# tprelle/janusgraph

Measured on AMD Instinct MI355X. Metric: GTEPS for PageRank iter + BFS, RMAT-24/26, 1/2/4/8 GPUs; % of HBM peak, higher is better.
Workload: dtype f64

## Files before the change

janusgraph_amd/csrc/jg_api.cpp:

```cpp
#include <dlfcn.h>
#include <execinfo.h>

#include <algorithm>
#include <atomic>
#include <cstdlib>
#include <cstring>
#include <limits>
#include <map>
#include <mutex>

#include "jg_cache.h"
#include "jg_internal.h"
#include "jg_labelset.h"

namespace jg {

namespace {
thread_local std::string g_last_error;
}

void rccl_check(ncclResult_t r, const char* what) {
    if (r != ncclSuccess) fail(JG_ERR_RCCL, std::string(what) + ": " + ncclGetErrorString(r));
}

// ... 595 lines not shown
    bool sealed = false;
    jg::DevBuf<int64_t> lab;
    int64_t ml = 0;
};

using jg::Error;

#define JG_GUARD_BEGIN try {
#define JG_GUARD_END                                       \
    jg::dev_cache_sync();                                  \
    return JG_OK;                                          \
    }                                                      \
    catch (const Error& e) {                               \
        jg::g_last_error_set(e.what());                    \
        return e.code;                                     \
    }                                                      \
    catch (const std::bad_alloc&) {                        \
        jg::g_last_error_set("host allocation failed");    \
        return JG_ERR_OOM;                                 \
    }                                                      \
    catch (const std::exception& e) {                      \
        jg::g_last_error_set(e.what());                    \
        return JG_ERR_HIP;                                 \
    }

namespace jg {
void g_last_error_set(const char* m) { g_last_error = m ? m : ""; }
}

#define JG_ARG(cond, msg) \
    if (!(cond)) jg::fail(JG_ERR_ARG, msg)

extern "C" {

int jg_abi_version(void) { return JG_ABI_VERSION; }

int jg_tune_set(const char* key, int64_t value) {
    JG_GUARD_BEGIN
    JG_ARG(key, "null key");
    const std::string k(key);
    jg::Tune& t = jg::tune();
    if (k == "dev_poison_probe") {
        jg::dev_poison_probe(value);
        return JG_OK;
    }
    struct Knob {
        const char* name;
        int* field;
        int64_t lo, hi;
    };
    const Knob knobs[] = {
        {"pull_split", &t.pull_split, 0, 1},
        {"halo", &t.halo, 0, 1},
        {"bfs_alpha", &t.bfs_alpha, 1, 1000000},
        {"dobfs_alpha", &t.dobfs_alpha, 1, 1000000},
        {"bfs_beta", &t.bfs_beta, 1, 1000000},
        {"bfs_narrow", &t.bfs_narrow, 0, 1},
        {"nb_alpha", &t.nb_alpha, 1, 1000000},
        {"nb_first", &t.nb_first, 4, 4096},
        {"cc_push", &t.cc_push, 0, 1},
        {"msbfs_sparse", &t.msbfs_sparse, 0, 1},
        {"msbfs_td", &t.msbfs_td, 0, 2},
        {"cc_first", &t.cc_first, 1, 64},
        {"msbfs_skip", &t.msbfs_skip, 0, 1},
        {"msbfs_exit", &t.msbfs_exit, 0, 2},
        {"msbfs_td_rowapply", &t.msbfs_td_rowapply, 0, 1024},
        {"msbfs_td_noprobe", &t.msbfs_td_noprobe, 0, 1000},
        {"msbfs_scan_queue", &t.msbfs_scan_queue, 0, 1001},
        {"msbfs_exit_first", &t.msbfs_exit_first, 1, 256},
        {"msbfs_exit_live", &t.msbfs_exit_live, 0, 1000},
        {"cc_uf", &t.cc_uf, 0, 1},
        {"cc_uf_sharded", &t.cc_uf_sharded, 0, 1},
        {"cc_uf_search", &t.cc_uf_search, 0, 1},
        {"cc_sparse", &t.cc_sparse, 0, 1},
        {"msbfs_split", &t.msbfs_split, 0, 1},
        {"sharded_bfs", &t.sharded_bfs, 0, 1},
        {"bfs_td_split", &t.bfs_td_split, 0, 2},
        {"bfs_td_split_levels", &t.bfs_td_split_levels, 0, 0xffff},
        {"bfs_batch0", &t.bfs_batch0, 1, 64},
        {"bfs_grid_mult", &t.bfs_grid_mult, 1, 64},
        {"bfs_grid", &t.bfs_grid, 64, 65536},
        {"bfs_tail_grid", &t.bfs_tail_grid, 0, 65536},
        {"merge_temporal", &t.merge_temporal, 0, 2},
        {"sd_delta", &t.sd_delta, -1, 1 << 30},
        {"sd_dist32", &t.sd_dist32, 0, 2},
    };
    for (const Knob& kn : knobs) {
        if (k != kn.name) continue;
        if (value < kn.lo || value > kn.hi)
            jg::fail(JG_ERR_ARG, k + " must be in [" + std::to_string(kn.lo) + ", " + std::to_string(kn.hi) + "]");
        *kn.field = (int)value;
        return JG_OK;
    }
    if (k.rfind("band", 0) == 0 && k.size() == 9 && k[4] >= '0' && k[4] <= '3' &&
        (k.substr(5) == "_deg" || k.substr(5) == "_bit" || k.substr(5) == "_sub")) {
        const int i = k[4] - '0';
        if (k.substr(5) == "_deg") {
            JG_ARG(value >= -1, "band degree must be >= 0 (0: unused) or -1 (automatic)");
            t.band_deg[i] = value;
        } else if (k.substr(5) == "_bit") {
            JG_ARG(value == 0 || (value >= 3 && value <= 8), "band bits must be 0 (automatic) or in [3, 8]");
            t.band_bits[i] = value == 0 ? -1 : (int)value;
        } else {
            JG_ARG(value >= 1 && value <= 256 && (value & (value - 1)) == 0, "band sub-slices must be a power of two in [1, 256]");
            int b = 0;
            while ((1 << b) < value) ++b;
            t.band_bits[i] = b;
        }
    } else if (k.size() == 12 && k.compare(0, 11, "merge_stage") == 0 && k[11] >= '0' && k[11] <= '3') {
        JG_ARG(value == -1 || value == 0 || value == 64 || value == 128 || value == 256 || value == 512,
               "merge_stage<i> must be -1 (automatic), 0, 64, 128, 256 or 512");
        t.merge_stage[k[11] - '0'] = (int)value;
    } else if (k == "bfs_td_split_min" || k == "bfs_td_split_max") {
        JG_ARG(value >= 1 && value <= INT32_MAX, "bfs_td_split_min / _max must be in [1, 2^31)");
        (k == "bfs_td_split_min" ? t.bfs_td_split_min : t.bfs_td_split_max) = value;
    } else if (k == "merge_pack") {
        JG_ARG(value == 0 || value == 1 || value == 24, "merge_pack must be 0 (32 bits), 1 (automatic) or 24 (at least 24)");
        t.merge_pack = (int)value;
    } else if (k == "pull_unroll" || k == "pull_nt" || k == "pull_lds" || k == "light_lds" || k == "slice_lds" ||
               k == "pull_short" || k == "pull_overlap" || k == "bfs_persistent") {
    } else {
        jg::fail(JG_ERR_ARG, "unknown tuning key: " + k);
    }
    JG_GUARD_END
}

const char* jg_last_error(void) { return jg::g_last_error.c_str(); }

int jg_comm_unique_id(void* out) {
    JG_GUARD_BEGIN
    JG_ARG(out, "null output");
    ncclUniqueId id;
    jg::rccl_check(ncclGetUniqueId(&id), "ncclGetUniqueId");
    static_assert(sizeof(ncclUniqueId) == JG_UNIQUE_ID_BYTES, "unique id size");
    std::memcpy(out, &id, sizeof id);
    JG_GUARD_END
}

int jg_ctx_create(const int* devices, int ndev, jg_ctx** out) {
    JG_GUARD_BEGIN
    JG_ARG(out && devices && ndev > 0, "jg_ctx_create: need devices and an output pointer");
    *out = nullptr;
    int count = 0;
    JG_HIP(hipGetDeviceCount(&count));
    for (int i = 0; i < ndev; ++i)
        JG_ARG(devices[i] >= 0 && devices[i] < count, "jg_ctx_create: device ordinal out of range");
    auto ctx = std::make_unique<jg_ctx>();
    jg::Ctx& c = ctx->impl;
    c.devices.assign(devices, devices + ndev);
    bool all_same = true;
    for (int i = 1; i < ndev; ++i) all_same &= devices[i] == devices[0];
    c.logical = ndev > 1 && all_same;
    jg::vdev_refresh();
    jg::dev_poison_refresh();
    c.vdev = c.logical && jg::vdev_mode() != 0;
    if (ndev > 1 && !all_same) {
        std::vector<int> sorted(c.devices);
        std::sort(sorted.begin(), sorted.end());
        JG_ARG(std::adjacent_find(sorted.begin(), sorted.end()) == sorted.end(),
               "jg_ctx_create: mix of repeated and distinct devices");
    }
    for (int i = 0; i < ndev; ++i) {
        jg::DeviceGuard dg(c.devices[i]);
        hipStream_t s = nullptr;
        if (c.logical && i > 0) s = c.streams[0];
        else JG_HIP(hipStreamCreateWithFlags(&s, hipStreamNonBlocking));
// ... 804 lines not shown
```

janusgraph_amd/csrc/jg_internal.h:

```cpp
#pragma once

#include <algorithm>
#include <memory>
#include <atomic>
#include <mutex>
#include <functional>
#include <vector>

#include "jg_common.h"
#include "janusgpu.h"

#include <rccl/rccl.h>

namespace jg {

struct Csr {
    int64_t rows = 0;
    int64_t nnz = 0;
    DevBuf<int64_t> row_ptr;
    DevBuf<int32_t> col;
    DevBuf<int32_t> weight;
    mutable int64_t empty_from = -1;
    mutable DevBuf<int32_t> first_col;
    mutable long long wstat[4] = {0, 0, 0, 0};
// ... 404 lines not shown
void graph_neighbors(const Graph& g, int direction, const int64_t* rows, int64_t nrows, int64_t* off_out,
                     int64_t* nbr_out);
void shortest_distance_run(Graph& g, int64_t seed_vid, int max_depth, int64_t* dist_out);
using CcLabelHook = std::function<void(const int32_t* label, int64_t lrows)>;
void cc_run(Graph& g, int64_t* comp_out, int32_t* iterations_out, const CcLabelHook* labels_hook = nullptr);
void cc_census(Graph& g, int64_t min_population, int32_t* iterations_out, int64_t* components_out, int64_t* listed_out,
               int64_t* largest_out, double* census_ms_out);
void cc_census_read(Graph& g, int64_t first, int64_t count, int64_t* vid_out, int64_t* pop_out);
void cc_census_drop(Graph& g);
void cc_prepare_ranks(Graph& g);
struct CcRoots {
    int32_t* parent;
    const int32_t* rank;
    const int32_t* minr;
    int64_t ne;
};
int cc_root_eccentricity(Ctx& ctx, Shard& sh, const CcRoots& r, int32_t* depth, double* edges_out,
                         const std::function<void()>* after_start = nullptr, hipEvent_t end_ev = nullptr);
int cc_root_eccentricity_sharded(Graph& g, const CcRoots* roots, double* edges_out);
void bfs_buffers(Shard& sh);
const int32_t* bfs_first_col(Shard& sh, const Csr& c);
void region_mark(hipStream_t s, bool begin);
constexpr int kNarrowMax = 8;
struct NarrowRun {
    int levels = 0;
    float ms = 0;
    double entries = 0;
    double bytes = 0;
    double reached = 0;
};
NarrowRun narrow_bfs(Ctx& ctx, Shard& sh, const Csr& push, const Csr& pull, const int64_t* src, int ns, int max_depth,
                     int32_t* planes);
void combine_run(Graph& g, int direction, int combiner, int wrap32, const int64_t* init, int steps, int64_t* out,
                 uint8_t* received_out);

int allreduce_or(Graph& g, int flag);
void allreduce_sum_i64(Graph& g, int64_t* vals, int n);
uint64_t allreduce_or_u64(Graph& g, uint64_t v);

bool pull_split_launches();
bool debug_plan();
bool debug_bfs();

struct Tune {
    int pull_split = 1;
    int64_t band_deg[4] = {96, -1, -1, 0};
    int band_bits[4] = {-1, -1, -1, 3};
    int halo = 1;
    int bfs_alpha = 14;
    int dobfs_alpha = 30;
    int bfs_beta = 24;
    int bfs_narrow = 1;
    int nb_alpha = 30;
    int nb_first = 16;
    int cc_push = 1;
    int msbfs_sparse = 1;
    int msbfs_td = 1;
    int cc_first = 1;
    int msbfs_skip = 1;
    int msbfs_exit = 1;
    int msbfs_td_rowapply = 4;
    int msbfs_td_noprobe = 2;
    int msbfs_scan_queue = 50;
    int msbfs_exit_first = 16;
    int msbfs_exit_live = 950;
    int cc_uf = 1;
    int cc_uf_sharded = 1;
    int cc_uf_search = 1;
    int cc_sparse = 1;
    int msbfs_split = 1;
    int sharded_bfs = 1;
    int bfs_td_split = 2;
    int bfs_td_split_levels = 2;
    int64_t bfs_td_split_min = 65536;
    int64_t bfs_td_split_max = 1 << 20;
    int bfs_batch0 = 10;
    int bfs_grid_mult = 4;
    int bfs_grid = 8192;
    int bfs_tail_grid = 64;
    int sd_dist32 = 1;
    int sd_delta = -1;
    int merge_temporal = 1;
    int merge_stage[4] = {-1, -1, -1, -1};
    int merge_pack = 1;
};
Tune& tune();
void host_allgather(Ctx& c, const void* in, void* out, size_t bytes);
void host_exchange(Ctx& c, const std::vector<int>& speer, const std::vector<const void*>& sbuf,
                   const std::vector<size_t>& sbytes, const std::vector<int>& rpeer, const std::vector<void*>& rbuf,
                   const std::vector<size_t>& rbytes);
int device_cu_count();

bool prof_enabled(const Ctx& c);
void prof_record_start(Ctx& c, Shard& sh);
void prof_record_stop(Ctx& c, Shard& sh, int units = 1);
void prof_collect(Ctx& c, Graph& g);
void exch_record(Ctx& c, Shard& sh);
void prof_discard_exchanges(Graph& g);
struct ExchTimer {
    Graph& g;
    explicit ExchTimer(Graph& gr);
    ~ExchTimer();
};

}

struct jg_ctx {
    jg::Ctx impl;
};
struct jg_graph {
    jg::Graph impl;
    explicit jg_graph(jg::Ctx* c) {
        impl.ctx = c;
        c->live.fetch_add(1);
    }
    ~jg_graph() { impl.ctx->live.fetch_sub(1); }
    jg_graph(const jg_graph&) = delete;
    jg_graph& operator=(const jg_graph&) = delete;
};
```

janusgraph_amd/csrc/jg_pull.h:

```cpp
#pragma once

#include <type_traits>

#include "jg_internal.h"
#include "jg_prim.h"

namespace jg {

struct PullArgs {
    const int64_t* __restrict__ row_ptr;
    const int32_t* __restrict__ col;
    const int64_t* __restrict__ chunk_row;
    const int64_t* __restrict__ chunk_begin;
    const int64_t* __restrict__ chunk_end;
    const int64_t* __restrict__ hub_chunk_ptr;
    int64_t num_chunks;
    int64_t num_hub_rows;
    int64_t class_row_begin[kNumClasses];
    int64_t class_row_end[kNumClasses];
    int64_t class_block_begin[kNumClasses + 1];
    int64_t block_offset;
    int64_t skip_rows;
    int runs;
    int64_t run_begin[kRunMax + 1];
// ... 147 lines not shown
    for (int k = 1; k < kNumClasses; ++k)
        if (b >= a.class_block_begin[k + 1]) c = k + 1;
    const int64_t lb = b - a.class_block_begin[c];
    switch (c) {
        case 1: pull_rows_class<Op, 64, U>(a, op, gather, c, lb, tid); break;
        case 2: pull_rows_class<Op, 32, U>(a, op, gather, c, lb, tid); break;
        case 3: pull_rows_class<Op, 16, U>(a, op, gather, c, lb, tid); break;
        case 4: pull_rows_class<Op, 8, U>(a, op, gather, c, lb, tid); break;
        case 5: pull_rows_class<Op, 4, U>(a, op, gather, c, lb, tid); break;
        case 6: pull_rows_class<Op, 2, U>(a, op, gather, c, lb, tid); break;
        case 7: pull_rows_class<Op, 1, U>(a, op, gather, c, lb, tid); break;
        default: pull_rows_empty<Op>(a, op, lb, tid); break;
    }
}

template <class Op, int U>
__device__ __forceinline__ void pull_block(const PullArgs& a, const Op& op, typename Op::T* __restrict__ hub_partial,
                                           int64_t b) {
    using T = typename Op::T;
    if (b < a.num_chunks) {
        __shared__ T red[kBlock / kWave];
        const int64_t j0 = a.chunk_begin[b], j1 = a.chunk_end[b];
        const int64_t crow = a.chunk_row[b];
        T acc = (crow >= a.skip_rows && op.active(crow)) ? fold_strided<Op, U>(op, a.col, j0 + threadIdx.x, j1, kBlock)
                                                         : op.identity();
#pragma unroll
        for (int o = kWave / 2; o > 0; o >>= 1) acc = op.combine(acc, op.shfl_xor(acc, o));
        if (lane_id() == 0) red[wave_id()] = acc;
        __syncthreads();
        if (threadIdx.x == 0) {
            T t = red[0];
#pragma unroll
            for (int w = 1; w < kBlock / kWave; ++w) t = op.combine(t, red[w]);
            hub_partial[b] = t;
        }
        return;
    }
    pull_block_rows<Op, U>(a, op, GlobalGather<Op>{op}, b, (int)threadIdx.x);
}

template <class Op, int U>
__global__ __launch_bounds__(kBlock) void pull_kernel(PullArgs a, Op op, typename Op::T* __restrict__ hub_partial) {
    pull_block<Op, U>(a, op, hub_partial, (int64_t)blockIdx.x + a.block_offset);
}

template <class Op>
__global__ void pull_hub_finalize_kernel(PullArgs a, Op op, const typename Op::T* __restrict__ hub_partial) {
    using T = typename Op::T;
    for (int64_t h = (int64_t)blockIdx.x * blockDim.x + threadIdx.x; h < a.num_hub_rows;
         h += (int64_t)gridDim.x * blockDim.x) {
        const int64_t c0 = a.hub_chunk_ptr[h], c1 = a.hub_chunk_ptr[h + 1];
        if (a.chunk_row[c0] < a.skip_rows) continue;
        T acc = op.identity();
        for (int64_t k = c0; k < c1; ++k) acc = op.combine(acc, hub_partial[k]);
        op.finalize(a.chunk_row[c0], acc);
    }
}

constexpr int kMergeThreads = 1024;
constexpr int kMergeWaves = kMergeThreads / kWave;
constexpr int kMergeEpl = kMergeTask / kWave;
constexpr int kMergeLdsBytes = 160 * 1024;

struct MergeArgs {
    const uint4* __restrict__ pack_a;
    const uint32_t* __restrict__ pack_b;
    const uint8_t* __restrict__ heads;
    const int32_t* __restrict__ meta;
    const int64_t* __restrict__ sub_begin;
    const int64_t* __restrict__ sub_end;
    const int64_t* __restrict__ sub_base;
    int64_t tasks;
    int bits;
    int stage;
    const uint32_t* __restrict__ live;
};

struct HotSegs {
    int32_t hs = 0;
    int tbits = 31;
    int nseg = 1;
};

template <class Op, bool MSEG = true>
struct SliceGather {
    using T = typename Op::T;
    const Op& op;
    lds_ptr<const T> lds;
    uint32_t hg;
    int sb;
    int bits;
    uint32_t hmask, h;
    uint32_t idcell;
    __device__ __forceinline__ bool is_hot(uint32_t loc) const {
        if constexpr (!MSEG) return loc < (hg << 4);
        return ((loc >> 4) & ((1u << sb) - 1u)) < hg;
    }
    __device__ __forceinline__ T hot(uint32_t loc, bool valid) const {
        if constexpr (!MSEG) return lds[valid && loc < (hg << 4) ? loc : idcell];
        const uint32_t g = loc >> 4, j = g & ((1u << sb) - 1u), seg = g >> sb;
        return lds[valid && j < hg ? (((seg * hg + j) << 4) | (loc & 15u)) : idcell];
    }
    __device__ __forceinline__ int32_t col(uint32_t loc) const {
        const uint32_t x = (loc >> 4) << bits;
        const uint32_t hx = (x ^ (x >> 8) ^ (x >> 16) ^ (x >> 24)) & hmask;
        return (int32_t)(((x | (h ^ hx)) << 4) | (loc & 15u));
    }
    __device__ __forceinline__ T cold(uint32_t loc, bool valid, bool lds_on) const {
        T v = op.identity();
        if (valid && !(lds_on && is_hot(loc))) v = op.gather(col(loc));
        return v;
    }
};

template <int W>
__device__ __forceinline__ uint32_t unpack_entry(const uint32_t (&d)[W / 4], int u) {
    const int o = W * u, i = o >> 5, sh = o & 31;
    uint32_t v = d[i] >> sh;
    if (sh + W > 32) v |= d[i + 1] << (32 - sh);
    if constexpr (W < 32) v &= (1u << W) - 1u;
    return v;
}

template <class T>
__device__ __forceinline__ T lane_up(T v, int lane, int d) {
    static_assert(sizeof(T) % 4 == 0, "whole dwords");
    int w[sizeof(T) / 4];
    __builtin_memcpy(w, &v, sizeof(T));
    const int addr = ((lane - d) & (kWave - 1)) << 2;
#pragma unroll
    for (size_t i = 0; i < sizeof(T) / 4; ++i) w[i] = __builtin_amdgcn_ds_bpermute(addr, w[i]);
    __builtin_memcpy(&v, w, sizeof(T));
    return v;
}

template <class Op, class = void>
struct op_task_live : std::false_type {};
template <class Op>
struct op_task_live<Op, std::void_t<decltype(Op::kTaskLive)>> : std::bool_constant<Op::kTaskLive> {};

template <class Op, bool LDS, int PW, bool MSEG = false>
__global__ __launch_bounds__(kMergeThreads) void pull_merge_kernel(MergeArgs a, Op op, typename Op::T* __restrict__ partial,
                                                                   typename Op::T* __restrict__ carry, HotSegs hs,
                                                                   int temporal) {
    using T = typename Op::T;
    extern __shared__ __align__(16) unsigned char merge_lds[];
    const int S = 1 << a.bits;
    const int xs = S < kXcds ? S : kXcds;
    const int rep = kXcds / xs;
    const int per = S / xs;
    const int w = (int)(blockIdx.x >> 3), W = (int)(gridDim.x >> 3);
    const int xcd = (int)(blockIdx.x & (kXcds - 1));
    const int wave = threadIdx.x / kWave, lane = threadIdx.x % kWave;
    lds_ptr<T> hotv = (lds_ptr<T>)merge_lds;
    const int gshift = 4 + a.bits;
    const int hg = hs.hs >> gshift;
    const int nl = hs.nseg * hg;
    lds_ptr<T> stg = hotv + (nl * 16 + 1) + wave * (a.stage + 1);
    lds_ptr<uint32_t> tctr = (lds_ptr<uint32_t>)(hotv + (nl * 16 + 1) + kMergeWaves * (a.stage + 1));
    const int rounds = temporal ? per : 1;
    const uint32_t hmask = (1u << a.bits) - 1u;
    auto image_line = [&](int seg, int j, int hh) {
        const int64_t grp = ((int64_t)seg << (hs.tbits - gshift)) + j;
        return (grp << a.bits) + (int64_t)(hh ^ (sub_hash(grp << gshift) & hmask));
    };
    for (int rd = 0; rd < rounds; ++rd) {
    const int h = (xcd % xs) | ((temporal ? rd : w % per) << 3);
    const int64_t g = (int64_t)(temporal ? w : w / per) * rep + xcd / xs;
    const int64_t G = (int64_t)(temporal ? W : W / per) * rep;
    if constexpr (LDS) {
        if (rd > 0) __syncthreads();
        constexpr int kStage = 8;
        constexpr int kUnit = 16 / (int)sizeof(T);
        static_assert(16 % sizeof(T) == 0 && kUnit <= 16, "16-byte staging units");
        const unsigned char* src = reinterpret_cast<const unsigned char*>(op.vec());
        const int units = nl * 16 / kUnit;
        using u4 = uint32_t __attribute__((ext_vector_type(4)));
        lds_ptr<u4> hv4 = (lds_ptr<u4>)merge_lds;
        for (int q0 = 0; q0 < units; q0 += kStage * kMergeThreads) {
            u4 buf[kStage];
#pragma unroll
            for (int u = 0; u < kStage; ++u) {
                const int q = q0 + u * kMergeThreads + (int)threadIdx.x;
                const int i = q * kUnit, sg = i >> 4;
                int seg = 0, j = sg;
                if (hs.nseg > 1) {
                    seg = sg / hg;
                    j = sg - seg * hg;
                }
                buf[u] = u4{0, 0, 0, 0};
                if (q < units)
                    buf[u] = *reinterpret_cast<const u4*>(src + (image_line(seg, j, h) * 16 + (i & 15)) * (int64_t)sizeof(T));
            }
#pragma unroll
            for (int u = 0; u < kStage; ++u) {
                const int q = q0 + u * kMergeThreads + (int)threadIdx.x;
                if (q < units) hv4[q] = buf[u];
            }
        }
        if (threadIdx.x == 0) {
            hotv[nl * 16] = op.identity();
            *tctr = 0u;
        }
        __syncthreads();
    }
    const SliceGather<Op, MSEG> lg{op,       hotv, (uint32_t)hg, hs.tbits - gshift, a.bits, (1u << a.bits) - 1u, (uint32_t)h,
                             (uint32_t)nl * 16u};
    const int64_t base = a.sub_base[h];
    const int64_t ntask = a.sub_base[h + 1] - base;
    const int64_t hbegin = a.sub_begin[h], hend = a.sub_end[h];
    constexpr bool dyn = LDS;
    const int64_t grot = (g + rd) % G;
    auto task_of = [&](int64_t j) { return j * G + grot; };
    auto grab = [&]() -> int64_t {
        uint32_t j = 0;
        if (lane == 0) j = __hip_atomic_fetch_add(tctr, 1u, __ATOMIC_RELAXED, __HIP_MEMORY_SCOPE_WORKGROUP);
        return task_of((int64_t)__builtin_amdgcn_readfirstlane(j));
    };
    int64_t jstat = wave;
    auto advance = [&]() -> int64_t {
        if (dyn) return grab();
        jstat += kMergeWaves;
        return task_of(jstat);
    };
    auto dead = [&](int64_t kk) -> bool {
        if constexpr (!op_task_live<Op>::value) return false;
        if (a.live == nullptr || kk >= ntask) return false;
        const uint64_t tt = (uint64_t)(base + kk);
        const uint32_t wd = __builtin_amdgcn_readfirstlane(a.live[tt >> 5]);
        return ((wd >> (tt & 31)) & 1u) == 0;
    };
    int64_t k = dyn ? grab() : task_of(jstat);
    while (dead(k)) k = advance();
    if (k >= ntask) continue;
    static_assert(kMergeEpl == 8, "a lane chunk is 8 entries");
    constexpr int DB = PW / 4 - 4;
    auto chunk = [&](int64_t kk) { return (hbegin >> 3) + kk * kWave + lane; };
    auto meta_idx = [&](int64_t kk) { return 2 * (base + kk) + (lane & 1); };
    auto head_idx = [&](int64_t kk) { return (base + kk) * kWave + lane; };
    auto ld = [](const auto* p) { return *p; };
    using v4u = uint32_t __attribute__((ext_vector_type(4)));
    using v2u = uint32_t __attribute__((ext_vector_type(2)));
    auto load_chunk = [&](int64_t kk, uint32_t (&d)[PW / 4]) {
        const int64_t x = chunk(kk);
        const v4u va = ld(reinterpret_cast<const v4u*>(a.pack_a) + x);
        d[0] = va.x, d[1] = va.y, d[2] = va.z, d[3] = va.w;
        if constexpr (DB == 1) {
            d[4] = ld(a.pack_b + x);
        } else if constexpr (DB == 2) {
            const v2u vb = ld(reinterpret_cast<const v2u*>(a.pack_b) + x);
            d[4] = vb.x, d[5] = vb.y;
        } else {
            const v4u vb = ld(reinterpret_cast<const v4u*>(a.pack_b) + x);
            d[4] = vb.x, d[5] = vb.y, d[6] = vb.z, d[7] = vb.w;
        }
    };
    uint32_t cd[PW / 4];
    load_chunk(k, cd);
    uint32_t hb = ld(a.heads + head_idx(k));
    int32_t mw = ld(a.meta + meta_idx(k));
    for (;;) {
        const int64_t t = base + k;
        const int64_t e0 = hbegin + k * kMergeTask;
        const int n = (int)min((int64_t)kMergeTask, hend - e0);
        uint32_t loc[kMergeEpl];
#pragma unroll
        for (int u = 0; u < kMergeEpl; ++u) loc[u] = unpack_entry<PW>(cd, u);
        const int32_t j0 = __builtin_amdgcn_readlane(mw, 0);
        const bool carry_in = __builtin_amdgcn_readlane(mw, 1) != 0;
        const uint32_t hbc = hb;
        T v[kMergeEpl];
        if constexpr (LDS) {
            T vg[kMergeEpl], vl[kMergeEpl];
#pragma unroll
            for (int u = 0; u < kMergeEpl; ++u) vl[u] = lg.hot(loc[u], kMergeEpl * lane + u < n);
#pragma unroll
            for (int u = 0; u < kMergeEpl; ++u) vg[u] = lg.cold(loc[u], kMergeEpl * lane + u < n, true);
#pragma unroll
            for (int u = 0; u < kMergeEpl; ++u) v[u] = op.combine(vl[u], vg[u]);
        } else {
#pragma unroll
            for (int u = 0; u < kMergeEpl; ++u) v[u] = lg.cold(loc[u], kMergeEpl * lane + u < n, false);
        }
        int64_t kn = advance();
        while (dead(kn)) kn = advance();
        if (kn < ntask) {
            load_chunk(kn, cd);
            hb = ld(a.heads + head_idx(kn));
            mw = ld(a.meta + meta_idx(kn));
        }
        static_assert(kMergeEpl < 16, "a lane's head count has 4 bits");
        const uint32_t cnt = (uint32_t)__builtin_popcount(hbc);
        int hbase = 0;
        int H = 0;
#pragma unroll
        for (int b = 0; b < 4; ++b) {
            const uint64_t cb = __ballot((cnt >> b) & 1u);
            hbase += (int)__builtin_amdgcn_mbcnt_hi((uint32_t)(cb >> 32), __builtin_amdgcn_mbcnt_lo((uint32_t)cb, 0u)) << b;
            H += __builtin_popcountll(cb) << b;
        }
        const bool valid_lane = kMergeEpl * lane < n;
        const bool staged = LDS && H <= a.stage;
        const uint64_t hm = __ballot(hbc != 0u);
        const uint64_t hml = hm << (kWave - 1 - lane);
        const int gap = hml ? __builtin_clzll(hml) : kWave;
        const int reach = min(lane, gap);
        const int in_h = hbase - 1;
        auto store_partial = [&](int64_t j, T val) { partial[j] = val; };
        auto scan_in = [&](T x) -> T {
#pragma unroll
            for (int d = 1; d < kWave; d <<= 1) {
                const T xu = lane_up(x, lane, d);
                if (reach >= d) x = op.combine(xu, x);
            }
            return lane_up(x, lane, 1);
        };
        auto fold_direct = [&]() {
            auto emit = [&](int hh, T val) {
                if (hh == 0 && carry_in) carry[t] = val;
                else store_partial(j0 + hh, val);
            };
            const int fh = hbc ? __builtin_ctz(hbc) : kMergeEpl;
            T pre = op.identity(), run = op.identity();
            int run_h = hbase - 1;
#pragma unroll
            for (int u = 0; u < kMergeEpl; ++u) {
                if (u < fh) {
                    pre = u == 0 ? v[u] : op.combine(pre, v[u]);
                } else if ((hbc >> u) & 1u) {
                    if (u > fh) emit(run_h, run);
                    run = v[u];
                    ++run_h;
                } else {
                    run = op.combine(run, v[u]);
                }
            }
            const T in_x = scan_in(fh < kMergeEpl ? run : pre);
            if (valid_lane) {
                if (lane > 0 && fh < kMergeEpl) emit(in_h, fh > 0 ? op.combine(in_x, pre) : in_x);
                if (kMergeEpl * (lane + 1) >= n) {
                    if (fh < kMergeEpl) emit(run_h, run);
                    else emit(in_h, lane > 0 ? op.combine(in_x, pre) : pre);
                }
            }
        };
        auto fold_staged = [&]() {
            const int dump = a.stage;
            bool seen = (hbc & 1u) != 0u;
            int slot = in_h + (int)(hbc & 1u);
            T acc = v[0], pre = op.identity();
#pragma unroll
            for (int u = 1; u < kMergeEpl; ++u) {
                const bool head = ((hbc >> u) & 1u) != 0u;
                stg[head && seen ? slot : dump] = acc;
                pre = head && !seen ? acc : pre;
                const T sum = op.combine(acc, v[u]);
                acc = head ? v[u] : sum;
                slot += head ? 1 : 0;
                seen = seen || head;
            }
            pre = seen ? pre : acc;
            const T in_x = scan_in(acc);
            const T joined = op.combine(in_x, pre);
            stg[valid_lane && lane > 0 && seen ? in_h : dump] = (hbc & 1u) ? in_x : joined;
            const bool last = valid_lane && kMergeEpl * (lane + 1) >= n;
            const T whole = lane > 0 ? joined : pre;
            stg[last ? (seen ? slot : in_h) : dump] = seen ? acc : whole;
            __builtin_amdgcn_fence(__ATOMIC_RELEASE, "wavefront");
            __builtin_amdgcn_wave_barrier();
            __builtin_amdgcn_fence(__ATOMIC_ACQUIRE, "wavefront");
            for (int i = lane; i < H; i += kWave) {
                const T val = stg[i];
                if (i == 0 && carry_in) carry[t] = val;
                else store_partial(j0 + i, val);
            }
            __builtin_amdgcn_fence(__ATOMIC_RELEASE, "wavefront");
            __builtin_amdgcn_wave_barrier();
            __builtin_amdgcn_fence(__ATOMIC_ACQUIRE, "wavefront");
        };
        if constexpr (LDS) {
            if (staged) fold_staged();
            else fold_direct();
        } else {
            fold_direct();
        }
        if (kn >= ntask) break;
        k = kn;
    }
    }
}

constexpr int kMaxBands = 4;
struct FixupBands {
    const int32_t* meta[kMaxBands];
    int64_t task_begin[kMaxBands + 1];
    int64_t part_off[kMaxBands], carry_off[kMaxBands];
    int n;
};
template <class Op>
__global__ void pull_merge_fixup_kernel(FixupBands fb, Op op, typename Op::T* __restrict__ split_partial) {
    using T = typename Op::T;
    for (int64_t x = (int64_t)blockIdx.x * blockDim.x + threadIdx.x; x < fb.task_begin[fb.n];
         x += (int64_t)gridDim.x * blockDim.x) {
        int b = 0;
        while (x >= fb.task_begin[b + 1]) ++b;
        const int64_t t = x - fb.task_begin[b], tasks = fb.task_begin[b + 1] - fb.task_begin[b];
        const int32_t* __restrict__ meta = fb.meta[b];
        T* __restrict__ partial = split_partial + fb.part_off[b];
        const T* __restrict__ carry = split_partial + fb.carry_off[b];
        const int64_t tp = t > 0 ? t - 1 : 0, tn = t + 1 < tasks ? t + 1 : t;
        const int32_t f = meta[2 * t + 1], j = meta[2 * t];
        const int32_t pf = meta[2 * tp + 1], pj = meta[2 * tp];
        const int32_t nf = meta[2 * tn + 1], nj = meta[2 * tn];
        const T c = carry[t], cn = carry[tn];
        if (!f || (t > 0 && pf && pj == j)) continue;
        T acc = op.combine(partial[j], c);
        if (tn != t && nf && nj == j) {
            acc = op.combine(acc, cn);
            for (int64_t u = t + 2; u < tasks && meta[2 * u + 1] && meta[2 * u] == j; ++u) acc = op.combine(acc, carry[u]);
        }
        partial[j] = acc;
    }
}

struct FinalizeBands {
    const uint2* sub_word[kMaxBands];
    int64_t row_begin[kMaxBands];
    int64_t row_end[kMaxBands];
    int64_t part_off[kMaxBands];
    int bits[kMaxBands];
    int n;
};
template <class Op>
__device__ __forceinline__ void slice_finalize_row(int64_t r, const Op& op, const FinalizeBands& fb,
                                                   const typename Op::T* __restrict__ partial) {
    using T = typename Op::T;
    int b = 0;
    while (b < fb.n - 1 && r >= fb.row_end[b]) ++b;
    const int64_t NR = fb.row_end[b] - fb.row_begin[b], i = r - fb.row_begin[b];
    const int64_t W = (NR + 31) / 32, wi = i >> 5;
    const uint32_t below = (1u << (i & 31)) - 1u, me = 1u << (i & 31);
    const int S = 1 << fb.bits[b];
    const uint2* __restrict__ sw = fb.sub_word[b];
    const T* __restrict__ part = partial + fb.part_off[b];
    T acc = op.identity();
    bool first = true;
    uint2 wc[8], wn[8];
    auto load_words = [&](int h0, uint2 (&wd)[8]) {
#pragma unroll
        for (int u = 0; u < 8; ++u)
            wd[u] = h0 + u < S ? sw[(int64_t)(h0 + u) * W + wi] : make_uint2(0u, 0u);
    };
    load_words(0, wc);
    for (int h0 = 0; h0 < S; h0 += 8) {
        int32_t j[8];
        T v[8];
#pragma unroll
        for (int u = 0; u < 8; ++u) j[u] = (wc[u].x & me) ? (int32_t)wc[u].y + __popc(wc[u].x & below) : -1;
        if (h0 + 8 < S) load_words(h0 + 8, wn);
#pragma unroll
        for (int u = 0; u < 8; ++u) v[u] = j[u] >= 0 ? part[j[u]] : op.identity();
#pragma unroll
        for (int u = 0; u < 8; ++u)
            if (j[u] >= 0) {
                acc = first ? v[u] : op.combine(acc, v[u]);
                first = false;
            }
#pragma unroll
        for (int u = 0; u < 8; ++u) wc[u] = wn[u];
    }
    op.finalize(r, acc);
}

template <class Op>
__global__ void pull_slice_finalize_kernel(int64_t row0, int64_t rows, Op op, FinalizeBands fb,
                                           const typename Op::T* __restrict__ partial) {
    for (int64_t r = row0 + (int64_t)blockIdx.x * blockDim.x + threadIdx.x; r < rows; r += (int64_t)gridDim.x * blockDim.x)
        slice_finalize_row(r, op, fb, partial);
}

template <class Op, int U>
__global__ __launch_bounds__(kBlock) void pull_light_finalize_kernel(PullArgs a, Op op,
                                                                     typename Op::T* __restrict__ hub_partial,
                                                                     FinalizeBands fb,
                                                                     const typename Op::T* __restrict__ partial,
                                                                     int64_t split_rows, int64_t fin_blocks,
                                                                     int64_t fin_row0) {
    const int64_t b = blockIdx.x;
    if (b < fin_blocks) {
        const int64_t r = fin_row0 + b * kBlock + threadIdx.x;
        if (r < split_rows) slice_finalize_row<Op>(r, op, fb, partial);
        return;
    }
    pull_block<Op, U>(a, op, hub_partial, b - fin_blocks + a.block_offset);
}


template <class Op>
void launch_pull(const Csr& csr, const PullPlan& plan, const Op& op, typename Op::T* hub_partial, hipStream_t s,
                 Ctx* prof_ctx = nullptr, Shard* prof_shard = nullptr, typename Op::T* split_partial = nullptr,
                 bool skip_empty = false, const uint32_t* const* task_live = nullptr, int64_t caller_rows = 0) {
    using T = typename Op::T;
    const bool split = tune().pull_split && plan.split_rows > 0 && split_partial != nullptr;
    if (task_live != nullptr && !op_task_live<Op>::value)
        fail(JG_ERR_UNSUPPORTED, "launch_pull: this Op does not declare kTaskLive");
    size_t band0 = 0;
    if (caller_rows > 0) {
        while (band0 < plan.bands.size() && plan.bands[band0]->row_end <= caller_rows) ++band0;
        if (!split || band0 == 0 || plan.bands[band0 - 1]->row_end != caller_rows)
            fail(JG_ERR_UNSUPPORTED, "launch_pull: caller rows must end a prefix of the split bands");
    }
    PullArgs a = make_pull_args(csr, plan, split);
    if (skip_empty) a.class_block_begin[kNumClasses] = a.class_block_begin[kZeroClass];
    const int64_t blocks = a.class_block_begin[kNumClasses];
    if (prof_ctx) prof_record_start(*prof_ctx, *prof_shard);
    if (split) {
        static bool attr = false;
        if (!attr) {
            JG_HIP(hipFuncSetAttribute((const void*)pull_merge_kernel<Op, true, 20>,
                                       hipFuncAttributeMaxDynamicSharedMemorySize, kMergeLdsBytes));
            JG_HIP(hipFuncSetAttribute((const void*)pull_merge_kernel<Op, true, 24>,
                                       hipFuncAttributeMaxDynamicSharedMemorySize, kMergeLdsBytes));
            JG_HIP(hipFuncSetAttribute((const void*)pull_merge_kernel<Op, true, 32>,
                                       hipFuncAttributeMaxDynamicSharedMemorySize, kMergeLdsBytes));
            JG_HIP(hipFuncSetAttribute((const void*)pull_merge_kernel<Op, true, 20, true>,
                                       hipFuncAttributeMaxDynamicSharedMemorySize, kMergeLdsBytes));
            JG_HIP(hipFuncSetAttribute((const void*)pull_merge_kernel<Op, true, 24, true>,
                                       hipFuncAttributeMaxDynamicSharedMemorySize, kMergeLdsBytes));
            JG_HIP(hipFuncSetAttribute((const void*)pull_merge_kernel<Op, true, 32, true>,
                                       hipFuncAttributeMaxDynamicSharedMemorySize, kMergeLdsBytes));
            attr = true;
        }
        for (size_t bi = band0; bi < plan.bands.size(); ++bi) {
            const SliceBand& bd = *plan.bands[bi];
            if (bd.tasks == 0) continue;
            int stage = tune().merge_stage[std::min<size_t>(bi, 3)];
            if (stage < 0) {
                const double heads = (double)bd.subrows / (double)std::max<int64_t>(bd.tasks, 1);
                stage = 128;
                while (stage < 4.0 * heads && stage < 256) stage *= 2;
            }
            MergeArgs ma{bd.pack_a.get(), bd.pack_b.get(), bd.heads.get(), bd.meta.get(), bd.sub_begin.get(),
                         bd.sub_end.get(), bd.sub_base.get(), bd.tasks, bd.bits, stage,
                         task_live ? task_live[bi] : nullptr};
            T* part = split_partial + bd.part_off;
            T* carry = split_partial + bd.carry_off;
            const int64_t S = 1ll << bd.bits, gsz = 16 * S;
            const unsigned grid = (unsigned)std::max<int64_t>(S, (int64_t)device_cu_count() / S * S);
            const int64_t stage_bytes = (int64_t)kMergeWaves * (stage + 1) * (int64_t)sizeof(T);
            const int64_t hot_max = (int64_t)((kMergeLdsBytes - stage_bytes - 16) / (int64_t)sizeof(T) - 16) * S;
            HotSegs hs;
            hs.tbits = plan.seg_tbits;
            hs.nseg = plan.nseg;
            const int64_t seg_cap = plan.nseg == 1 ? plan.col_space : (1ll << plan.seg_tbits) - gsz;
            hs.hs = plan.lds_ok ? (int32_t)(std::min<int64_t>(hot_max / plan.nseg, seg_cap) / gsz * gsz) : 0;
            const int temporal = tune().merge_temporal == 2 || (tune().merge_temporal == 1 && plan.temporal);
            const size_t lds = hs.hs > 0 ? (size_t)(hs.nseg * (hs.hs / S) + 1) * sizeof(T) + (size_t)stage_bytes + 16 : 0;
            auto go = [&](auto kern) { kern<<<grid, kMergeThreads, lds, s>>>(ma, op, part, carry, hs, temporal); };
            if (hs.hs > 0 && hs.nseg > 1) {
                if (bd.width == 20) go(pull_merge_kernel<Op, true, 20, true>);
                else if (bd.width == 24) go(pull_merge_kernel<Op, true, 24, true>);
                else go(pull_merge_kernel<Op, true, 32, true>);
            } else if (hs.hs > 0) {
                if (bd.width == 20) go(pull_merge_kernel<Op, true, 20>);
                else if (bd.width == 24) go(pull_merge_kernel<Op, true, 24>);
                else go(pull_merge_kernel<Op, true, 32>);
            } else {
                if (bd.width == 20) go(pull_merge_kernel<Op, false, 20>);
                else if (bd.width == 24) go(pull_merge_kernel<Op, false, 24>);
                else go(pull_merge_kernel<Op, false, 32>);
            }
            JG_LAUNCH_CHECK();
        }
        FixupBands fx{};
        for (size_t bi = band0; bi < plan.bands.size(); ++bi) {
            const auto& bp = plan.bands[bi];
            if (fx.n == kMaxBands) fail(JG_ERR_UNSUPPORTED, "too many split bands");
            fx.meta[fx.n] = bp->meta.get();
            fx.part_off[fx.n] = bp->part_off;
            fx.carry_off[fx.n] = bp->carry_off;
            fx.task_begin[fx.n + 1] = fx.task_begin[fx.n] + bp->tasks;
            ++fx.n;
        }
        if (fx.task_begin[fx.n] > 0) {
            pull_merge_fixup_kernel<Op><<<grid_for(fx.task_begin[fx.n], kBlock, 0), kBlock, 0, s>>>(fx, op, split_partial);
            JG_LAUNCH_CHECK();
        }
    }
    auto launch = [&](unsigned grid) {
        pull_kernel<Op, 4><<<grid, kBlock, 0, s>>>(a, op, hub_partial);
        JG_LAUNCH_CHECK();
    };
    FinalizeBands fb{};
    if (split) {
        for (const auto& bp : plan.bands) {
            if (fb.n == kMaxBands) fail(JG_ERR_UNSUPPORTED, "too many split bands");
            fb.sub_word[fb.n] = bp->sub_word.get();
            fb.row_begin[fb.n] = bp->row_begin;
            fb.row_end[fb.n] = bp->row_end;
            fb.part_off[fb.n] = bp->part_off;
            fb.bits[fb.n] = bp->bits;
            ++fb.n;
        }
    }
    const bool fuse = split && !pull_split_launches();
    if (fuse) {
        const int64_t fin_blocks = (plan.split_rows - caller_rows + kBlock - 1) / kBlock;
        const unsigned grid = (unsigned)(fin_blocks + blocks);
        pull_light_finalize_kernel<Op, 4><<<grid, kBlock, 0, s>>>(a, op, hub_partial, fb, split_partial, plan.split_rows,
                                                                  fin_blocks, caller_rows);
        JG_LAUNCH_CHECK();
    } else if (pull_split_launches()) {
        for (int c = 0; c < kNumClasses; ++c) {
            const int64_t b0 = a.class_block_begin[c], b1 = a.class_block_begin[c + 1];
            if (b1 <= b0) continue;
            a.block_offset = b0;
            launch((unsigned)(b1 - b0));
        }
    } else if (blocks > 0) {
        launch((unsigned)blocks);
    }
    if (plan.num_hub_rows > 0 && !(split && plan.max_hub_row < plan.split_rows)) {
        pull_hub_finalize_kernel<Op><<<grid_for(plan.num_hub_rows), kBlock, 0, s>>>(a, op, hub_partial);
        JG_LAUNCH_CHECK();
    }
    if (split && !fuse) {
        if (plan.split_rows > caller_rows)
            pull_slice_finalize_kernel<Op><<<grid_for(plan.split_rows - caller_rows), kBlock, 0, s>>>(
                caller_rows, plan.split_rows, op, fb, split_partial);
        JG_LAUNCH_CHECK();
    }
    if (prof_ctx) prof_record_stop(*prof_ctx, *prof_shard);
}

}
```

Before: 386.6.

## Streamline merge kernel with byte offsets, uniform scalars, full-task specialization

The pull merge kernel now stores packed entries as pre-scaled byte offsets (O32) so gathers skip index-to-address multiplication. Task bounds and indices are forced onto scalar registers with readfirstlane. Full tasks get a specialized path with no per-lane validity checks. The next task's chunk is prefetched unconditionally using a clamped index, and sched barriers plus a later LDS combine reorder the instruction schedule. A merge_hot knob is added to cap the LDS hot region, and kernel dispatch is folded into a generic helper. The cost is more template instantiations and the need for the column space in bytes to fit in 32 bits.

Result: faster. 392.6 (median of 6 runs) (+1.5%).

```diff
diff --git a/janusgraph_amd/csrc/jg_api.cpp b/janusgraph_amd/csrc/jg_api.cpp
--- a/janusgraph_amd/csrc/jg_api.cpp
+++ b/janusgraph_amd/csrc/jg_api.cpp
@@ -701,6 +701,8 @@
         {"bfs_grid", &t.bfs_grid, 64, 65536},
         {"bfs_tail_grid", &t.bfs_tail_grid, 0, 65536},
         {"merge_temporal", &t.merge_temporal, 0, 2},
+        {"merge_hot", &t.merge_hot, -1, 1 << 30},
+        {"merge_off32", &t.merge_off32, 0, 1},
         {"sd_delta", &t.sd_delta, -1, 1 << 30},
         {"sd_dist32", &t.sd_dist32, 0, 2},
     };
diff --git a/janusgraph_amd/csrc/jg_internal.h b/janusgraph_amd/csrc/jg_internal.h
--- a/janusgraph_amd/csrc/jg_internal.h
+++ b/janusgraph_amd/csrc/jg_internal.h
@@ -510,6 +510,8 @@
     int sd_delta = -1;
     int merge_temporal = 1;
     int merge_stage[4] = {-1, -1, -1, -1};
+    int merge_hot = -1;
+    int merge_off32 = 1;
     int merge_pack = 1;
 };
 Tune& tune();
diff --git a/janusgraph_amd/csrc/jg_pull.h b/janusgraph_amd/csrc/jg_pull.h
--- a/janusgraph_amd/csrc/jg_pull.h
+++ b/janusgraph_amd/csrc/jg_pull.h
@@ -253,9 +253,12 @@
     int nseg = 1;
 };
 
-template <class Op, bool MSEG = true>
+template <class Op, bool MSEG = true, bool O32 = false>
 struct SliceGather {
     using T = typename Op::T;
+    static constexpr int LG = sizeof(T) == 4 ? 2 : sizeof(T) == 8 ? 3 : 4;
+    static_assert(sizeof(T) == (1u << LG), "4-, 8- or 16-byte values");
+    static constexpr int SH = O32 ? LG : 0;
     const Op& op;
     lds_ptr<const T> lds;
     uint32_t hg;
@@ -263,34 +266,73 @@
     int bits;
     uint32_t hmask, h;
     uint32_t idcell;
-    __device__ __forceinline__ bool is_hot(uint32_t loc) const {
-        if constexpr (!MSEG) return loc < (hg << 4);
-        return ((loc >> 4) & ((1u << sb) - 1u)) < hg;
-    }
-    __device__ __forceinline__ T hot(uint32_t loc, bool valid) const {
-        if constexpr (!MSEG) return lds[valid && loc < (hg << 4) ? loc : idcell];
-        const uint32_t g = loc >> 4, j = g & ((1u << sb) - 1u), seg = g >> sb;
-        return lds[valid && j < hg ? (((seg * hg + j) << 4) | (loc & 15u)) : idcell];
-    }
-    __device__ __forceinline__ int32_t col(uint32_t loc) const {
-        const uint32_t x = (loc >> 4) << bits;
+    __device__ __forceinline__ T lds_at(uint32_t e) const {
+        if constexpr (O32) return *(lds_ptr<const T>)((lds_ptr<const unsigned char>)lds + e);
+        return lds[e];
+    }
+    __device__ __forceinline__ bool is_hot(uint32_t e) const {
+        if constexpr (!MSEG) return e < idcell;
+        return ((e >> (4 + SH)) & ((1u << sb) - 1u)) < hg;
+    }
+    template <bool FULL>
+    __device__ __forceinline__ T hot(uint32_t e, bool valid) const {
+        if constexpr (!MSEG) {
+            const uint32_t i = min(e, idcell);
+            if constexpr (FULL) return lds_at(i);
+            return lds_at(valid ? i : idcell);
+        }
+        const uint32_t g = e >> (4 + SH), j = g & ((1u << sb) - 1u), seg = g >> sb;
+        const bool take = FULL ? j < hg : valid && j < hg;
+        return lds_at(take ? (((seg * hg + j) << (4 + SH)) | (e & (15u << SH))) : idcell);
+    }
+    __device__ __forceinline__ uint32_t line(uint32_t e) const {
+        const uint32_t x = (e >> (4 + SH)) << bits;
         const uint32_t hx = (x ^ (x >> 8) ^ (x >> 16) ^ (x >> 24)) & hmask;
-        return (int32_t)(((x | (h ^ hx)) << 4) | (loc & 15u));
-    }
-    __device__ __forceinline__ T cold(uint32_t loc, bool valid, bool lds_on) const {
+        return x | (h ^ hx);
+    }
+    __device__ __forceinline__ T load(uint32_t e) const {
+        if constexpr (O32) {
+            const uint32_t off = (line(e) << (4 + LG)) | (e & (15u << LG));
+            return *reinterpret_cast<const T*>(reinterpret_cast<const unsigned char*>(op.vec()) + off);
+        }
+        return op.gather((int32_t)((line(e) << 4) | (e & 15u)));
+    }
+    template <bool FULL>
+    __device__ __forceinline__ T cold(uint32_t e, bool valid, bool lds_on) const {
+        if constexpr (FULL) {
+            if (!lds_on) return load(e);
+        }
         T v = op.identity();
-        if (valid && !(lds_on && is_hot(loc))) v = op.gather(col(loc));
+        const bool c = !(lds_on && is_hot(e));
+        if (FULL ? c : valid && c) v = load(e);
         return v;
     }
 };
 
-template <int W>
+template <int W, int SH = 0>
 __device__ __forceinline__ uint32_t unpack_entry(const uint32_t (&d)[W / 4], int u) {
     const int o = W * u, i = o >> 5, sh = o & 31;
-    uint32_t v = d[i] >> sh;
-    if (sh + W > 32) v |= d[i + 1] << (32 - sh);
-    if constexpr (W < 32) v &= (1u << W) - 1u;
+    static_assert(W + SH <= 32 || W == 32, "a scaled entry fits a dword (W = 32: by launch_pull's gate)");
+    uint32_t v;
+    if (sh >= SH) {
+        v = d[i] >> (sh - SH);
+        if (sh + W > 32) v |= d[i + 1] << (32 - sh + SH);
+    } else {
+        v = d[i] << (SH - sh);
+    }
+    if constexpr (W < 32) v &= ((1u << W) - 1u) << SH;
     return v;
+}
+
+__device__ __forceinline__ int uniform32(int x) { return __builtin_amdgcn_readfirstlane(x); }
+__device__ __forceinline__ int64_t uniform64(int64_t x) {
+    const uint32_t lo = (uint32_t)__builtin_amdgcn_readfirstlane((int)(uint32_t)x);
+    const uint32_t hi = (uint32_t)__builtin_amdgcn_readfirstlane((int)(uint32_t)((uint64_t)x >> 32));
+    return (int64_t)(((uint64_t)hi << 32) | lo);
+}
+
+__device__ __forceinline__ bool uniform_less64(int64_t a, int64_t b) {
+    return __builtin_amdgcn_readfirstlane((int)((uint64_t)(a - b) >> 32)) < 0;
 }
 
 template <class T>
@@ -310,7 +352,7 @@
 template <class Op>
 struct op_task_live<Op, std::void_t<decltype(Op::kTaskLive)>> : std::bool_constant<Op::kTaskLive> {};
 
-template <class Op, bool LDS, int PW, bool MSEG = false>
+template <class Op, bool LDS, int PW, bool MSEG = false, bool O32 = false>
 __global__ __launch_bounds__(kMergeThreads) void pull_merge_kernel(MergeArgs a, Op op, typename Op::T* __restrict__ partial,
                                                                    typename Op::T* __restrict__ carry, HotSegs hs,
                                                                    int temporal) {
@@ -336,9 +378,9 @@
         return (grp << a.bits) + (int64_t)(hh ^ (sub_hash(grp << gshift) & hmask));
     };
     for (int rd = 0; rd < rounds; ++rd) {
-    const int h = (xcd % xs) | ((temporal ? rd : w % per) << 3);
+    const int h = uniform32((xcd % xs) | ((temporal ? rd : w % per) << 3));
     const int64_t g = (int64_t)(temporal ? w : w / per) * rep + xcd / xs;
-    const int64_t G = (int64_t)(temporal ? W : W / per) * rep;
+    const int64_t G = uniform64((int64_t)(temporal ? W : W / per) * rep);
     if constexpr (LDS) {
         if (rd > 0) __syncthreads();
         constexpr int kStage = 8;
@@ -375,13 +417,14 @@
         }
         __syncthreads();
     }
-    const SliceGather<Op, MSEG> lg{op,       hotv, (uint32_t)hg, hs.tbits - gshift, a.bits, (1u << a.bits) - 1u, (uint32_t)h,
-                             (uint32_t)nl * 16u};
-    const int64_t base = a.sub_base[h];
-    const int64_t ntask = a.sub_base[h + 1] - base;
-    const int64_t hbegin = a.sub_begin[h], hend = a.sub_end[h];
+    using Gather = SliceGather<Op, MSEG, O32>;
+    const Gather lg{op, hotv, (uint32_t)hg, hs.tbits - gshift, a.bits, (1u << a.bits) - 1u, (uint32_t)h,
+                    ((uint32_t)nl * 16u) << Gather::SH};
+    const int64_t base = uniform64(a.sub_base[h]);
+    const int64_t ntask = uniform64(a.sub_base[h + 1]) - base;
+    const int64_t hbegin = uniform64(a.sub_begin[h]), hend = uniform64(a.sub_end[h]);
     constexpr bool dyn = LDS;
-    const int64_t grot = (g + rd) % G;
+    const int64_t grot = uniform64((g + rd) % G);
     auto task_of = [&](int64_t j) { return j * G + grot; };
     auto grab = [&]() -> int64_t {
         uint32_t j = 0;
@@ -392,7 +435,7 @@
     auto advance = [&]() -> int64_t {
         if (dyn) return grab();
         jstat += kMergeWaves;
-        return task_of(jstat);
+        return uniform64(task_of(jstat));
     };
     auto dead = [&](int64_t kk) -> bool {
         if constexpr (!op_task_live<Op>::value) return false;
@@ -401,65 +444,64 @@
         const uint32_t wd = __builtin_amdgcn_readfirstlane(a.live[tt >> 5]);
         return ((wd >> (tt & 31)) & 1u) == 0;
     };
-    int64_t k = dyn ? grab() : task_of(jstat);
+    int64_t k = dyn ? grab() : uniform64(task_of(jstat));
     while (dead(k)) k = advance();
     if (k >= ntask) continue;
     static_assert(kMergeEpl == 8, "a lane chunk is 8 entries");
     constexpr int DB = PW / 4 - 4;
-    auto chunk = [&](int64_t kk) { return (hbegin >> 3) + kk * kWave + lane; };
-    auto meta_idx = [&](int64_t kk) { return 2 * (base + kk) + (lane & 1); };
-    auto head_idx = [&](int64_t kk) { return (base + kk) * kWave + lane; };
-    auto ld = [](const auto* p) { return *p; };
+    auto chunk0 = [&](int64_t kk) { return (hbegin >> 3) + kk * kWave; };
+    auto meta0 = [&](int64_t kk) { return 2 * (base + kk); };
+    auto head0 = [&](int64_t kk) { return (base + kk) * kWave; };
+    const uint32_t ulane = (uint32_t)lane;
     using v4u = uint32_t __attribute__((ext_vector_type(4)));
     using v2u = uint32_t __attribute__((ext_vector_type(2)));
     auto load_chunk = [&](int64_t kk, uint32_t (&d)[PW / 4]) {
-        const int64_t x = chunk(kk);
-        const v4u va = ld(reinterpret_cast<const v4u*>(a.pack_a) + x);
+        const int64_t x = chunk0(kk);
+        const v4u va = (reinterpret_cast<const v4u*>(a.pack_a) + x)[ulane];
         d[0] = va.x, d[1] = va.y, d[2] = va.z, d[3] = va.w;
         if constexpr (DB == 1) {
-            d[4] = ld(a.pack_b + x);
+            d[4] = (a.pack_b + x)[ulane];
         } else if constexpr (DB == 2) {
-            const v2u vb = ld(reinterpret_cast<const v2u*>(a.pack_b) + x);
+            const v2u vb = (reinterpret_cast<const v2u*>(a.pack_b) + x)[ulane];
             d[4] = vb.x, d[5] = vb.y;
         } else {
-            const v4u vb = ld(reinterpret_cast<const v4u*>(a.pack_b) + x);
+            const v4u vb = (reinterpret_cast<const v4u*>(a.pack_b) + x)[ulane];
             d[4] = vb.x, d[5] = vb.y, d[6] = vb.z, d[7] = vb.w;
         }
     };
+    auto load_head = [&](int64_t kk) -> uint32_t { return (a.heads + head0(kk))[ulane]; };
+    auto load_meta = [&](int64_t kk) -> int32_t { return (a.meta + meta0(kk))[ulane & 1u]; };
     uint32_t cd[PW / 4];
     load_chunk(k, cd);
-    uint32_t hb = ld(a.heads + head_idx(k));
-    int32_t mw = ld(a.meta + meta_idx(k));
-    for (;;) {
+    uint32_t hb = load_head(k);
+    int32_t mw = load_meta(k);
+    int64_t kn = k;
+    auto run_task = [&](auto full_c) __attribute__((always_inline)) {
+        constexpr bool FULL = decltype(full_c)::value;
         const int64_t t = base + k;
-        const int64_t e0 = hbegin + k * kMergeTask;
-        const int n = (int)min((int64_t)kMergeTask, hend - e0);
+        const int n = FULL ? kMergeTask : (int)(hend - (hbegin + k * kMergeTask));
         uint32_t loc[kMergeEpl];
 #pragma unroll
-        for (int u = 0; u < kMergeEpl; ++u) loc[u] = unpack_entry<PW>(cd, u);
+        for (int u = 0; u < kMergeEpl; ++u) loc[u] = unpack_entry<PW, Gather::SH>(cd, u);
         const int32_t j0 = __builtin_amdgcn_readlane(mw, 0);
         const bool carry_in = __builtin_amdgcn_readlane(mw, 1) != 0;
         const uint32_t hbc = hb;
-        T v[kMergeEpl];
+        T v[kMergeEpl], vl[kMergeEpl];
         if constexpr (LDS) {
-            T vg[kMergeEpl], vl[kMergeEpl];
-#pragma unroll
-            for (int u = 0; u < kMergeEpl; ++u) vl[u] = lg.hot(loc[u], kMergeEpl * lane + u < n);
-#pragma unroll
-            for (int u = 0; u < kMergeEpl; ++u) vg[u] = lg.cold(loc[u], kMergeEpl * lane + u < n, true);
-#pragma unroll
-            for (int u = 0; u < kMergeEpl; ++u) v[u] = op.combine(vl[u], vg[u]);
-        } else {
-#pragma unroll
-            for (int u = 0; u < kMergeEpl; ++u) v[u] = lg.cold(loc[u], kMergeEpl * lane + u < n, false);
-        }
-        int64_t kn = advance();
+#pragma unroll
+            for (int u = 0; u < kMergeEpl; ++u) vl[u] = lg.template hot<FULL>(loc[u], kMergeEpl * lane + u < n);
+        }
+#pragma unroll
+        for (int u = 0; u < kMergeEpl; ++u) v[u] = lg.template cold<FULL>(loc[u], kMergeEpl * lane + u < n, LDS);
+        kn = advance();
         while (dead(kn)) kn = advance();
-        if (kn < ntask) {
-            load_chunk(kn, cd);
-            hb = ld(a.heads + head_idx(kn));
-            mw = ld(a.meta + meta_idx(kn));
-        }
+        {
+            const int64_t kc = uniform_less64(kn, ntask) ? kn : ntask - 1;
+            load_chunk(kc, cd);
+            hb = load_head(kc);
+            mw = load_meta(kc);
+        }
+        __builtin_amdgcn_sched_barrier(0);
         static_assert(kMergeEpl < 16, "a lane's head count has 4 bits");
         const uint32_t cnt = (uint32_t)__builtin_popcount(hbc);
         int hbase = 0;
@@ -470,7 +512,13 @@
             hbase += (int)__builtin_amdgcn_mbcnt_hi((uint32_t)(cb >> 32), __builtin_amdgcn_mbcnt_lo((uint32_t)cb, 0u)) << b;
             H += __builtin_popcountll(cb) << b;
         }
-        const bool valid_lane = kMergeEpl * lane < n;
+        __builtin_amdgcn_sched_barrier(0);
+        if constexpr (LDS) {
+#pragma unroll
+            for (int u = 0; u < kMergeEpl; ++u) v[u] = op.combine(vl[u], v[u]);
+        }
+        const bool valid_lane = FULL || kMergeEpl * lane < n;
+        const bool last_lane = FULL ? lane == kWave - 1 : valid_lane && kMergeEpl * (lane + 1) >= n;
         const bool staged = LDS && H <= a.stage;
         const uint64_t hm = __ballot(hbc != 0u);
         const uint64_t hml = hm << (kWave - 1 - lane);
@@ -509,7 +557,7 @@
             const T in_x = scan_in(fh < kMergeEpl ? run : pre);
             if (valid_lane) {
                 if (lane > 0 && fh < kMergeEpl) emit(in_h, fh > 0 ? op.combine(in_x, pre) : in_x);
-                if (kMergeEpl * (lane + 1) >= n) {
+                if (last_lane) {
                     if (fh < kMergeEpl) emit(run_h, run);
                     else emit(in_h, lane > 0 ? op.combine(in_x, pre) : pre);
                 }
@@ -534,9 +582,8 @@
             const T in_x = scan_in(acc);
             const T joined = op.combine(in_x, pre);
             stg[valid_lane && lane > 0 && seen ? in_h : dump] = (hbc & 1u) ? in_x : joined;
-            const bool last = valid_lane && kMergeEpl * (lane + 1) >= n;
             const T whole = lane > 0 ? joined : pre;
-            stg[last ? (seen ? slot : in_h) : dump] = seen ? acc : whole;
+            stg[last_lane ? (seen ? slot : in_h) : dump] = seen ? acc : whole;
             __builtin_amdgcn_fence(__ATOMIC_RELEASE, "wavefront");
             __builtin_amdgcn_wave_barrier();
             __builtin_amdgcn_fence(__ATOMIC_ACQUIRE, "wavefront");
@@ -555,7 +602,12 @@
         } else {
             fold_direct();
         }
-        if (kn >= ntask) break;
+    };
+    for (;;) {
+        const bool full = !uniform_less64(hend - (hbegin + k * kMergeTask), kMergeTask);
+        if (__builtin_expect(full, 1)) run_task(std::true_type{});
+        else run_task(std::false_type{});
+        if (!uniform_less64(kn, ntask)) break;
         k = kn;
     }
     }
@@ -686,20 +738,27 @@
     const int64_t blocks = a.class_block_begin[kNumClasses];
     if (prof_ctx) prof_record_start(*prof_ctx, *prof_shard);
     if (split) {
+        auto with_kernel = [](int width, bool image, bool mseg, bool o32, auto&& f) {
+            auto widths = [&](auto l, auto m, auto o) {
+                constexpr bool L = decltype(l)::value, M = decltype(m)::value, O = decltype(o)::value;
+                if (width == 20) f(pull_merge_kernel<Op, L, 20, M, O>);
+                else if (width == 24) f(pull_merge_kernel<Op, L, 24, M, O>);
+                else f(pull_merge_kernel<Op, L, 32, M, O>);
+            };
+            constexpr std::true_type yes{};
+            constexpr std::false_type no{};
+            if (image && mseg) o32 ? widths(yes, yes, yes) : widths(yes, yes, no);
+            else if (image) o32 ? widths(yes, no, yes) : widths(yes, no, no);
+            else o32 ? widths(no, no, yes) : widths(no, no, no);
+        };
         static bool attr = false;
         if (!attr) {
-            JG_HIP(hipFuncSetAttribute((const void*)pull_merge_kernel<Op, true, 20>,
-                                       hipFuncAttributeMaxDynamicSharedMemorySize, kMergeLdsBytes));
-            JG_HIP(hipFuncSetAttribute((const void*)pull_merge_kernel<Op, true, 24>,
-                                       hipFuncAttributeMaxDynamicSharedMemorySize, kMergeLdsBytes));
-            JG_HIP(hipFuncSetAttribute((const void*)pull_merge_kernel<Op, true, 32>,
-                                       hipFuncAttributeMaxDynamicSharedMemorySize, kMergeLdsBytes));
-            JG_HIP(hipFuncSetAttribute((const void*)pull_merge_kernel<Op, true, 20, true>,
-                                       hipFuncAttributeMaxDynamicSharedMemorySize, kMergeLdsBytes));
-            JG_HIP(hipFuncSetAttribute((const void*)pull_merge_kernel<Op, true, 24, true>,
-                                       hipFuncAttributeMaxDynamicSharedMemorySize, kMergeLdsBytes));
-            JG_HIP(hipFuncSetAttribute((const void*)pull_merge_kernel<Op, true, 32, true>,
-                                       hipFuncAttributeMaxDynamicSharedMemorySize, kMergeLdsBytes));
+            for (int width : {20, 24, 32})
+                for (int v = 0; v < 4; ++v)
+                    with_kernel(width, true, (v & 1) != 0, (v & 2) != 0, [](auto kern) {
+                        JG_HIP(hipFuncSetAttribute((const void*)kern, hipFuncAttributeMaxDynamicSharedMemorySize,
+                                                   kMergeLdsBytes));
+                    });
             attr = true;
         }
         for (size_t bi = band0; bi < plan.bands.size(); ++bi) {
@@ -724,23 +783,14 @@
             hs.tbits = plan.seg_tbits;
             hs.nseg = plan.nseg;
             const int64_t seg_cap = plan.nseg == 1 ? plan.col_space : (1ll << plan.seg_tbits) - gsz;
-            hs.hs = plan.lds_ok ? (int32_t)(std::min<int64_t>(hot_max / plan.nseg, seg_cap) / gsz * gsz) : 0;
+            int64_t hot = plan.lds_ok ? std::min<int64_t>(hot_max / plan.nseg, seg_cap) : 0;
+            if (tune().merge_hot >= 0) hot = std::min<int64_t>(hot, tune().merge_hot);
+            hs.hs = (int32_t)(hot / gsz * gsz);
+            const bool o32 = tune().merge_off32 != 0 && plan.col_space * (int64_t)sizeof(T) <= (1ll << 32);
             const int temporal = tune().merge_temporal == 2 || (tune().merge_temporal == 1 && plan.temporal);
             const size_t lds = hs.hs > 0 ? (size_t)(hs.nseg * (hs.hs / S) + 1) * sizeof(T) + (size_t)stage_bytes + 16 : 0;
             auto go = [&](auto kern) { kern<<<grid, kMergeThreads, lds, s>>>(ma, op, part, carry, hs, temporal); };
-            if (hs.hs > 0 && hs.nseg > 1) {
-                if (bd.width == 20) go(pull_merge_kernel<Op, true, 20, true>);
-                else if (bd.width == 24) go(pull_merge_kernel<Op, true, 24, true>);
-                else go(pull_merge_kernel<Op, true, 32, true>);
-            } else if (hs.hs > 0) {
-                if (bd.width == 20) go(pull_merge_kernel<Op, true, 20>);
-                else if (bd.width == 24) go(pull_merge_kernel<Op, true, 24>);
-                else go(pull_merge_kernel<Op, true, 32>);
-            } else {
-                if (bd.width == 20) go(pull_merge_kernel<Op, false, 20>);
-                else if (bd.width == 24) go(pull_merge_kernel<Op, false, 24>);
-                else go(pull_merge_kernel<Op, false, 32>);
-            }
+            with_kernel(bd.width, hs.hs > 0, hs.nseg > 1, o32, go);
             JG_LAUNCH_CHECK();
         }
         FixupBands fx{};
```
